# facebookresearch/generative-recommenders

Hardware: NVIDIA H100
Metric: user-seqs/sec HSTU-large L=8192 d=256 bf16 fwd+bwd (higher is better)
Workload: dtype bf16

## Files before the change

### generative_recommenders_b200/build.py

```python
import concurrent.futures
import importlib.util
import os
import shutil
import subprocess
import sys

HERE = os.path.dirname(os.path.abspath(__file__))
ROOT = os.path.dirname(HERE)
CSRC = os.path.join(HERE, "csrc")
OBJ = os.path.join(ROOT, "build", "hstu_b200")
LIB = os.path.join(HERE, "lib", "libhstu_b200.so")
SELFTEST_LIB = os.path.join(HERE, "lib", "libhstu_b200_selftest.so")
GEN = os.path.join(OBJ, "gen")
SELFTEST_SOURCES = ["wgmma_selftest.cu", "tmap.cu"]
SOURCES = ["api.cu", "attn_generic.cu", "attn_wgmma_fwd.cu", "attn_wgmma_bwd.cu", "attn_wgmma_fwd_e4m3.cu", "attn_wgmma_mixed_fwd.cu", "attn_wgmma_mixed_bwd.cu", "attn_fp16_operands.cu", "tmap.cu", "norm.cu", "norm_fast.cu", "jagged.cu", "position.cu", "sampled_softmax.cu", "jagged_bmm.cu"]
NVCC_FLAGS = [
    "-std=c++20", "-gencode", "arch=compute_90a,code=sm_90a", "-lineinfo", "-O3",
    "-Xcompiler", "-fPIC", "-Xcompiler", "-Wall", "-Xcudafe", "--diag_suppress=177",
]


def _nvcc() -> str:
    for cand in (os.environ.get("NVCC"), shutil.which("nvcc"), "/usr/local/cuda/bin/nvcc"):
        if cand and os.path.exists(cand):
            return cand
    raise RuntimeError("nvcc not found")


def _deps_mtime() -> float:
    paths = [os.path.join(CSRC, f) for f in os.listdir(CSRC)] + [os.path.join(ROOT, "include", "hstu_b200.h"), __file__,
# ... 64 lines not shown
```

### generative_recommenders_b200/csrc/attn_wgmma_bwd.cu

```cuda
#include "attn_wgmma_bwd.cuh"

namespace hstu {

template <int D, bool BF16>
__global__ void __launch_bounds__(kAttnThreads, 1) attn_bwd_wgmma_kernel(const __grid_constant__ BwdParams p) {
  bwd_key_tile<D, D, BF16, true>(p);
}

template <int D, bool BF16>
__global__ void __launch_bounds__(kAttnThreads, split_min_blocks(D)) attn_bwd_dkdv_wgmma_kernel(const __grid_constant__ BwdParams p) {
  bwd_key_tile<D, D, BF16, false>(p);
}

template <int D, bool BF16>
__global__ void __launch_bounds__(kAttnThreads, split_min_blocks(D)) attn_bwd_dq_wgmma_kernel(const __grid_constant__ BwdParams p) {
  bwd_dq_body<D, D, BF16>(p);
}

template <bool BF16>
__global__ void dq_convert_kernel(const float* __restrict__ acc, uint16_t* __restrict__ dq, long long rows, int heads, int D,
                                  long long row_stride, long long head_stride, float scale) {
  const long long nvec = rows * heads * (D / 8);
  for (long long idx = (long long)blockIdx.x * blockDim.x + threadIdx.x; idx < nvec; idx += (long long)gridDim.x * blockDim.x) {
    const int v = (int)(idx % (D / 8));
// ... 26 lines not shown
  hstu_attn_params q = p;
  if (q.out == nullptr) q.out = const_cast<void*>(q.q);
  q.o_row_stride = 8;
  q.o_head_stride = 8;
  return wgmma_bwd_supported(q);
}

static bool split_dq(const hstu_attn_params& p) {
  return p.dqk == 32 || p.dqk == 256 || p.dqk != p.dv || p.deterministic != 0;
}

static bool fp16_copies(const hstu_attn_params& p) { return p.dtype == HSTU_BF16 && p.dqk == 32 && p.dv == 32; }

size_t wgmma_workspace_bytes(const hstu_attn_params& p, bool bwd) {
  if (!bwd && p.delta_q_len > 0) return wgmma_delta_workspace_bytes(p);
  if (fp16_copies(p)) return fp16_operands_workspace_bytes(p, bwd);
  if (!bwd || split_dq(p)) return 0;
  return (size_t)p.total_rows * p.heads * p.dqk * sizeof(float);
}

template <int D, bool BF16, bool kSplit>
static int launch_bwd_wgmma(const hstu_attn_params& p, cudaStream_t st, const Fp16Operands* f16 = nullptr) {
  if constexpr (kSplit) {
    return launch_bwd_split<D, D, BF16>(p, st, attn_bwd_dkdv_wgmma_kernel<D, BF16>, attn_bwd_dq_wgmma_kernel<D, BF16>, f16);
  } else {
    using Cfg = BwdCfg<D, D, true>;
    const size_t need = wgmma_workspace_bytes(p, true);
    if (p.workspace == nullptr || p.workspace_bytes < need) {
      set_error("hstu_attn_bwd: workspace of %zu bytes required (got %zu)", need, p.workspace_bytes);
      return HSTU_ERR_WORKSPACE;
    }
    const BwdOperands o = bwd_operands(p, f16);
    BwdParams bp = bwd_params(p, f16);
    if (int e = make_tmap_rows_heads(&bp.tmQ, o.src[0], p.total_rows, p.heads, D, o.rs[0], o.hs[0], Cfg::BOX_COLS, Cfg::BQ)) return e;
    if (int e = make_tmap_rows_heads(&bp.tmK, o.src[1], p.total_rows, p.heads, D, o.rs[1], o.hs[1], Cfg::BOX_COLS, Cfg::BKV)) return e;
    if (int e = make_tmap_rows_heads(&bp.tmV, o.src[2], p.total_rows, p.heads, D, o.rs[2], o.hs[2], Cfg::BOX_COLS, Cfg::BKV)) return e;
    if (int e = make_tmap_rows_heads(&bp.tmDO, o.src[3], p.total_rows, p.heads, D, o.rs[3], o.hs[3], Cfg::BOX_COLS, Cfg::BQ)) return e;
    HSTU_CUDA_OK(cudaMemsetAsync(p.workspace, 0, need, st));
    auto kern = attn_bwd_wgmma_kernel<D, BF16>;
// ... 8 lines not shown
                                                         p.dq_row_stride, p.dq_head_stride, bp.dk_scale);
    HSTU_CUDA_OK(cudaGetLastError());
    return 0;
  }
}

int attn_wgmma_bwd(const hstu_attn_params& p, cudaStream_t st) {
  if (p.dqk != p.dv) return attn_wgmma_bwd_mixed(p, st);
  const bool bf = p.dtype == HSTU_BF16;
  const bool split = split_dq(p);
  switch (p.dqk) {
    case 32: {
      if (!bf) return launch_bwd_wgmma<32, false, true>(p, st);
      Fp16Operands f16;
      if (int e = fp16_operands_prepass(p, true, &f16, st)) return e;
      return launch_bwd_wgmma<32, false, true>(p, st, &f16);
    }
    case 64:
      if (split) return bf ? launch_bwd_wgmma<64, true, true>(p, st) : launch_bwd_wgmma<64, false, true>(p, st);
      return bf ? launch_bwd_wgmma<64, true, false>(p, st) : launch_bwd_wgmma<64, false, false>(p, st);
    case 128:
      if (split) return bf ? launch_bwd_wgmma<128, true, true>(p, st) : launch_bwd_wgmma<128, false, true>(p, st);
      return bf ? launch_bwd_wgmma<128, true, false>(p, st) : launch_bwd_wgmma<128, false, false>(p, st);
    case 256:
      return bf ? launch_bwd_wgmma<256, true, true>(p, st) : launch_bwd_wgmma<256, false, true>(p, st);
  }
  set_error("wgmma backward: unsupported head dim %d", p.dqk);
  return HSTU_ERR_UNSUPPORTED;
}

}
// ... 1 lines not shown
```

### generative_recommenders_b200/csrc/attn_wgmma_bwd.cuh

```cuda
#pragma once
#include <string.h>

#include <type_traits>

#include "attn_fp16_operands.cuh"
#include "attn_wgmma_qtile.cuh"
#include "common.cuh"
#include "internal.h"
#include "wgmma.cuh"

namespace hstu {
using namespace wg;

struct alignas(64) BwdParams {
  CUtensorMap tmQ, tmK, tmV, tmDO;
  SeqArgs seq;
  void* dk;
  void* dv;
  float* dq_acc;
  void* dq;
  long long dk_row_stride, dk_head_stride, dv_row_stride, dv_head_stride, dq_row_stride, dq_head_stride;
  float dv_scale;
  float dk_scale;
  const uint32_t* amax;
};

struct BwdScales {
  float c_s = 0.f, c_p = 1.f, c_d = 1.f;
  int e_dv = 0, e_dk = 0, e_dq = 0;
  __device__ __forceinline__ BwdScales(const BwdParams& p, int b, int h, int d) {
    c_s = p.seq.alpha_half;
    if (p.amax == nullptr) return;
    const OperandExps ex = operand_exps(p.amax + ((long long)b * p.seq.heads + h) * kAmaxSlots, 2.f * p.seq.alpha_half, d);
    c_s = ldexpf(p.seq.alpha_half, -(ex.q + ex.k));
    c_p = pow2f(ex.p);
    c_d = pow2f(ex.s - ex.v - ex.o);
    e_dv = -(ex.p + ex.o);
    e_dk = -(ex.s + ex.q);
    e_dq = -(ex.s + ex.k);
// ... 37 lines not shown
  uint64_t qd_full[4];
  uint32_t qd_free[4];
};

struct QTiles {
  int A, first, T;
  __device__ __forceinline__ int at(int i) const { return i < A ? i : first + (i - A); }
};

template <int DQK, int DV, bool BF16, bool FUSED_DQ>
__device__ __forceinline__ void bwd_key_tile(const BwdParams& p) {
  using Cfg = BwdCfg<DQK, DV, FUSED_DQ>;
  constexpr int SW = Cfg::SW, SWQ = Cfg::SWQ, SWV = Cfg::SWV, BQ = Cfg::BQ, NST = Cfg::STAGES;
  constexpr int NSL = Cfg::NSL, DNK = DQK / NSL, DNV = DV / NSL;
  static_assert(DNK % Cfg::BOX_COLS_Q == 0 && DNV % Cfg::BOX_COLS_V == 0, "a slice is whole boxes");
  const int b = blockIdx.z, h = blockIdx.y;
  const int n0 = (blockIdx.x / NSL) * Cfg::BKV;
  const int ck0 = (blockIdx.x % NSL) * DNK, cv0 = (blockIdx.x % NSL) * DNV;
  const long long row0 = load_index(p.seq.seq_offsets, p.seq.offsets_i64, b);
  int len = (int)(load_index(p.seq.seq_offsets, p.seq.offsets_i64, b + 1) - row0);
  if (len > p.seq.max_seq_len) {
    if (blockIdx.x == 0) {
      zero_rows(p.dk, 2, p.dk_row_stride, (long long)h * p.dk_head_stride, DQK, row0 + p.seq.max_seq_len, row0 + len);
      zero_rows(p.dv, 2, p.dv_row_stride, (long long)h * p.dv_head_stride, DV, row0 + p.seq.max_seq_len, row0 + len);
    }
    len = p.seq.max_seq_len;
  }
  if (n0 >= len) return;
  const int n_tgt = p.seq.num_targets ? (int)load_index(p.seq.num_targets, p.seq.targets_i64, b) : -1;
  const SeqMask msk = make_seq_mask(len, n_tgt, p.seq.win, p.seq.min_full, p.seq.ctx);
  const int nrows = min(Cfg::BKV, len - n0);
  QTiles qt;
  {
    int lo, hi, ctx_hi;
    q_range_for_kv_rows(msk, n0, n0 + nrows, &lo, &hi, &ctx_hi);
    qt.A = (ctx_hi + BQ - 1) / BQ;
    qt.first = max(lo / BQ, qt.A);
// ... 273 lines not shown
  static constexpr int STAGES = 3;
  static constexpr int OFF_Q = 0;
  static constexpr int OFF_DO = OFF_Q + Q_BYTES;
  static constexpr int OFF_K = OFF_DO + DO_BYTES;
  static constexpr int OFF_V = OFF_K + STAGES * K_BYTES;
  static constexpr int OFF_BAR = OFF_V + STAGES * V_BYTES;
  static constexpr int SMEM_BYTES = OFF_BAR + 256 + 1024;
  static_assert(SMEM_BYTES * split_min_blocks(DV) <= kSmemPerSm, "shared memory budget of split_min_blocks(dv) CTAs per SM");
};

template <int DQK, int DV, bool BF16>
__device__ __forceinline__ void bwd_dq_body(const BwdParams& p) {
  using Cfg = DqCfg<DQK, DV>;
  constexpr int SW = Cfg::SW, SWV = Cfg::SWV, BN = Cfg::BN, NST = Cfg::STAGES;
  constexpr bool kScaled = !BF16 && DQK == 32 && DV == 32;
  const int b = blockIdx.z, h = blockIdx.y;
  const int m0 = (int)(gridDim.x - 1 - blockIdx.x) * Cfg::BM;
  QTileSeq qs;
  if (!qtile_prologue<Cfg::BM, BN>(p.seq, b, h, m0, p.dq, p.dq_row_stride, p.dq_head_stride, DQK, &qs)) return;

  uint8_t* smem = dyn_smem_1k();
  KvRing<Cfg> ring{smem, &p.tmK, &p.tmV, h, qs.row0, qs.t0, qs.T};
  ring.init();
  const int tid = threadIdx.x, warp = tid >> 5, lane = tid & 31;
  if (tid == 0) {
    prefetch_tensormap(&p.tmQ);
    prefetch_tensormap(&p.tmK);
    prefetch_tensormap(&p.tmV);
    prefetch_tensormap(&p.tmDO);
    mbar_arrive_expect_tx(&ring.bars->q_full, Cfg::Q_BYTES + Cfg::DO_BYTES);
#pragma unroll
    for (int bx = 0; bx < imax(Cfg::NBOX, Cfg::NBOX_V); ++bx) {
      if (bx < Cfg::NBOX) tma_load_3d(smem + Cfg::OFF_Q + bx * Cfg::Q_BOX, &p.tmQ, &ring.bars->q_full, bx * Cfg::BOX_COLS, h, (int)(qs.row0 + m0));
      if (bx < Cfg::NBOX_V)
// ... 127 lines not shown
  bp.dq_acc = reinterpret_cast<float*>(p.workspace);
  bp.dq = p.dq;
  bp.dk_row_stride = p.dk_row_stride;
  bp.dk_head_stride = p.dk_head_stride;
  bp.dv_row_stride = p.dv_row_stride;
  bp.dv_head_stride = p.dv_head_stride;
  bp.dq_row_stride = p.dq_row_stride;
  bp.dq_head_stride = p.dq_head_stride;
  bp.dv_scale = 1.0f / (float)p.max_seq_len;
  bp.dk_scale = 0.5f * p.alpha / (float)p.max_seq_len;
  return bp;
}

template <int DQK, int DV, bool BF16>
int launch_bwd_split(const hstu_attn_params& p, cudaStream_t st, void (*kdkdv)(BwdParams), void (*kdq)(BwdParams),
                     const Fp16Operands* f16 = nullptr) {
  using Cfg = BwdCfg<DQK, DV, false>;
  const BwdOperands o = bwd_operands(p, f16);
  const int d[4] = {DQK, DQK, DV, DV};
  BwdParams bp = bwd_params(p, f16);
  if (int e = make_tmap_rows_heads(&bp.tmQ, o.src[0], p.total_rows, p.heads, d[0], o.rs[0], o.hs[0], Cfg::BOX_COLS_Q, Cfg::BQ)) return e;
  if (int e = make_tmap_rows_heads(&bp.tmK, o.src[1], p.total_rows, p.heads, d[1], o.rs[1], o.hs[1], Cfg::BOX_COLS, Cfg::BKV)) return e;
  if (int e = make_tmap_rows_heads(&bp.tmV, o.src[2], p.total_rows, p.heads, d[2], o.rs[2], o.hs[2], Cfg::BOX_COLS_V, Cfg::BKV)) return e;
  if (int e = make_tmap_rows_heads(&bp.tmDO, o.src[3], p.total_rows, p.heads, d[3], o.rs[3], o.hs[3], Cfg::BOX_COLS_V, Cfg::BQ)) return e;
  HSTU_CUDA_OK(cudaFuncSetAttribute(kdkdv, cudaFuncAttributeMaxDynamicSharedMemorySize, Cfg::SMEM_BYTES));
  const int key_ctas = (p.max_seq_len + Cfg::BKV - 1) / Cfg::BKV * Cfg::NSL;
  kdkdv<<<dim3(key_ctas, p.heads, p.batch), kAttnThreads, Cfg::SMEM_BYTES, st>>>(bp);
  HSTU_CUDA_OK(cudaGetLastError());
  using QC = DqCfg<DQK, DV>;
  if (int e = make_tmap_rows_heads(&bp.tmQ, o.src[0], p.total_rows, p.heads, d[0], o.rs[0], o.hs[0], QC::BOX_COLS, QC::BM)) return e;
  if (int e = make_tmap_rows_heads(&bp.tmK, o.src[1], p.total_rows, p.heads, d[1], o.rs[1], o.hs[1], QC::BOX_COLS, QC::BN)) return e;
  if (int e = make_tmap_rows_heads(&bp.tmV, o.src[2], p.total_rows, p.heads, d[2], o.rs[2], o.hs[2], QC::BOX_COLS_V, QC::BN)) return e;
  if (int e = make_tmap_rows_heads(&bp.tmDO, o.src[3], p.total_rows, p.heads, d[3], o.rs[3], o.hs[3], QC::BOX_COLS_V, QC::BM)) return e;
  HSTU_CUDA_OK(cudaFuncSetAttribute(kdq, cudaFuncAttributeMaxDynamicSharedMemorySize, QC::SMEM_BYTES));
  kdq<<<dim3((p.max_seq_len + QC::BM - 1) / QC::BM, p.heads, p.batch), kAttnThreads, QC::SMEM_BYTES, st>>>(bp);
  HSTU_CUDA_OK(cudaGetLastError());
  return 0;
}

}
```

### generative_recommenders_b200/csrc/attn_wgmma_fwd.cu

```cuda
#include "attn_wgmma_fwd.cuh"

namespace hstu {

template <int D, bool BF16>
__global__ void __launch_bounds__(kAttnThreads, kFwdMinBlocks<D>) attn_fwd_wgmma_kernel(const __grid_constant__ FwdParams p) {
  attn_fwd_wgmma_body<D, D, BF16, false>(p);
}
template <int D, bool BF16>
__global__ void __launch_bounds__(kAttnThreads, kFwdMinBlocks<D>) attn_fwd_delta_wgmma_kernel(const __grid_constant__ FwdParams p) {
  attn_fwd_wgmma_body<D, D, BF16, true>(p);
}

template <bool BF16>
__global__ void __launch_bounds__(256) delta_reduce_kernel(const float* __restrict__ part, void* out, long long rows, int heads, int d,
                                                            int chunks, long long o_row_stride, long long o_head_stride, float inv_n) {
  const long long plane = rows * heads * d, n4 = plane / 4;
  for (long long i = (long long)blockIdx.x * 256 + threadIdx.x; i < n4; i += (long long)gridDim.x * 256) {
    float4 a = reinterpret_cast<const float4*>(part)[i];
    for (int c = 1; c < chunks; ++c) {
      const float4 x = reinterpret_cast<const float4*>(part + c * plane)[i];
      a.x += x.x, a.y += x.y, a.z += x.z, a.w += x.w;
    }
    const long long e = i * 4, r = e / ((long long)heads * d), hc = e % ((long long)heads * d);
    const long long off = r * o_row_stride + (hc / d) * o_head_stride + hc % d;
// ... 43 lines not shown
    return false;
  return is_sm90();
}

int launch_delta_reduce(bool bf16, const float* part, void* out, long long rows, int heads, int d, int chunks,
                        long long o_row_stride, long long o_head_stride, float inv_n, cudaStream_t st) {
  const long long n4 = rows * heads * d / 4;
  const int blocks = (int)std::min<long long>((n4 + 255) / 256, kDeltaReduceBlocks);
  auto kern = bf16 ? delta_reduce_kernel<true> : delta_reduce_kernel<false>;
  kern<<<blocks, 256, 0, st>>>(part, out, rows, heads, d, chunks, o_row_stride, o_head_stride, inv_n);
  HSTU_CUDA_OK(cudaGetLastError());
  return 0;
}

template <int D, bool BF16, bool kDelta = false>
static int launch_fwd(const hstu_attn_params& p, cudaStream_t st, const Fp16Operands* f16 = nullptr) {
  auto kern = [] {
    if constexpr (kDelta) return attn_fwd_delta_wgmma_kernel<D, BF16>;
    else return attn_fwd_wgmma_kernel<D, BF16>;
  }();
  return launch_fwd_wgmma<D, D, BF16, kDelta>(p, st, kern, f16);
}

int attn_wgmma_fwd(const hstu_attn_params& p, cudaStream_t st) {
  if (p.dqk != p.dv) return attn_wgmma_fwd_mixed(p, st);
  const bool bf = p.dtype == HSTU_BF16;
  if (p.delta_q_len > 0) {
    switch (p.dqk) {
      case 32: return bf ? launch_fwd<32, true, true>(p, st) : launch_fwd<32, false, true>(p, st);
      case 64: return bf ? launch_fwd<64, true, true>(p, st) : launch_fwd<64, false, true>(p, st);
      case 128: return bf ? launch_fwd<128, true, true>(p, st) : launch_fwd<128, false, true>(p, st);
      case 256: return bf ? launch_fwd<256, true, true>(p, st) : launch_fwd<256, false, true>(p, st);
    }
  }
  switch (p.dqk) {
    case 32: {
      if (!bf) return launch_fwd<32, false>(p, st);
      Fp16Operands f16;
      if (int e = fp16_operands_prepass(p, false, &f16, st)) return e;
      return launch_fwd<32, false>(p, st, &f16);
    }
    case 64: return bf ? launch_fwd<64, true>(p, st) : launch_fwd<64, false>(p, st);
    case 128: return bf ? launch_fwd<128, true>(p, st) : launch_fwd<128, false>(p, st);
    case 256: return bf ? launch_fwd<256, true>(p, st) : launch_fwd<256, false>(p, st);
  }
  set_error("wgmma forward: unsupported head dim %d", p.dqk);
  return HSTU_ERR_UNSUPPORTED;
}

}
```

### generative_recommenders_b200/csrc/attn_wgmma_fwd.cuh

```cuda
#pragma once
#include <string.h>

#include <algorithm>
#include <type_traits>

#include "attn_fp16_operands.cuh"
#include "attn_wgmma_qtile.cuh"
#include "common.cuh"
#include "internal.h"
#include "wgmma.cuh"

namespace hstu {
using namespace wg;

struct alignas(64) FwdParams {
  CUtensorMap tmQ, tmK, tmV;
  SeqArgs seq;
  void* out;
  long long o_row_stride, o_head_stride;
  float inv_n;
  const uint32_t* amax;
  int delta;
  float* part;
};

template <int DQK, int DV = DQK>
struct FwdCfg {
  static constexpr int BM = 128;
  static constexpr int BN = 64;
  static constexpr int SW = swizzle_bytes(DQK), SWV = swizzle_bytes(DV);
  static constexpr int BOX_COLS = SW / 2;
  static constexpr int BOX_COLS_V = SWV / 2;
  static constexpr int Q_BOX = BM * SW;
  static constexpr int K_BOX = BN * SW;
  static constexpr int V_BOX = BN * SWV;
  static constexpr int Q_BYTES = BM * DQK * 2;
  static constexpr int K_BYTES = BN * DQK * 2;
  static constexpr int V_BYTES = BN * DV * 2;
// ... 14 lines not shown
  long long out_row, part_row;
  int rows;
};
template <int BM>
__device__ __forceinline__ DeltaRows delta_rows(const FwdParams& p) {
  const int m0 = (int)blockIdx.y * BM;
  const long long r = (long long)(blockIdx.x / p.seq.heads) * p.delta + m0;
  return {r, (long long)blockIdx.z * (gridDim.x / p.seq.heads) * p.delta + r, min(BM, p.delta - m0)};
}

template <int DQK, int DV, bool BF16, bool kDelta>
__device__ __forceinline__ void attn_fwd_wgmma_body(const FwdParams& p) {
  using Cfg = FwdCfg<DQK, DV>;
  constexpr int SW = Cfg::SW, SWV = Cfg::SWV, BN = Cfg::BN, NST = Cfg::STAGES;
  constexpr bool kMerge = DV <= 64;
  const int b = kDelta ? (int)blockIdx.x / p.seq.heads : (int)blockIdx.z, h = kDelta ? (int)blockIdx.x % p.seq.heads : (int)blockIdx.y;
  const int m0 = kDelta ? (int)blockIdx.y * Cfg::BM : (int)(gridDim.x - 1 - blockIdx.x) * Cfg::BM;
  QTileSeq qs;
  if constexpr (kDelta) {
    seq_rows(p.seq, b, &qs);
  } else if (!qtile_rows(p.seq, b, h, m0, p.out, p.o_row_stride, p.o_head_stride, DV, &qs)) {
    return;
  }
  const int p0 = kDelta ? qs.len - p.delta + m0 : m0;
  key_tiles<Cfg::BM, BN>(p.seq, b, p0, (kDelta ? p.delta : qs.len) - m0, &qs);
  if constexpr (kDelta) {
    const int per = (qs.T + (int)gridDim.z - 1) / (int)gridDim.z;
    qs.t0 += (int)blockIdx.z * per;
    qs.T = min(per, qs.T - (int)blockIdx.z * per);
    if (qs.T <= 0) {
      const DeltaRows dr = delta_rows<Cfg::BM>(p);
      for (int idx = threadIdx.x; idx < dr.rows * DV; idx += kAttnThreads) {
        if (gridDim.z > 1) p.part[((dr.part_row + idx / DV) * p.seq.heads + h) * DV + idx % DV] = 0.f;
        else reinterpret_cast<uint16_t*>(p.out)[(dr.out_row + idx / DV) * p.o_row_stride + (long long)h * p.o_head_stride + idx % DV] = 0;
      }
      return;
// ... 167 lines not shown
      for (int nb = 0; nb < DV / 8; ++nb) {
        float a = o[nb * 4 + hh * 2] * p.inv_n, c = o[nb * 4 + hh * 2 + 1] * p.inv_n;
        if (kScaled) a = scalbnf(a, e_out), c = scalbnf(c, e_out);
        *reinterpret_cast<uint32_t*>(orow + nb * 8 + 2 * t4) = out_bf16 ? pack_bf16x2(a, c) : pack_f16x2(a, c);
      }
    }
  }
}


int delta_chunks(const hstu_attn_params& p);
int launch_delta_reduce(bool bf16, const float* part, void* out, long long rows, int heads, int d, int chunks,
                        long long o_row_stride, long long o_head_stride, float inv_n, cudaStream_t st);

template <int DQK, int DV, bool BF16, bool kDelta>
int launch_fwd_wgmma(const hstu_attn_params& p, cudaStream_t st, void (*kern)(FwdParams), const Fp16Operands* f16 = nullptr) {
  using Cfg = FwdCfg<DQK, DV>;
  FwdParams fp;
  memset(&fp, 0, sizeof(fp));
  const int chunks = kDelta ? delta_chunks(p) : 1;
  if (chunks > 1) {
    const size_t need = wgmma_delta_workspace_bytes(p);
    if (p.workspace == nullptr || p.workspace_bytes < need) {
      set_error("hstu_attn_fwd: delta_q workspace of %zu bytes required (got %zu)", need, p.workspace_bytes);
      return HSTU_ERR_WORKSPACE;
    }
    fp.part = reinterpret_cast<float*>(p.workspace);
  }
  const long long q_rows = kDelta ? (long long)p.batch * p.delta_q_len : p.total_rows;
  if (f16) {
    const long long crs = (long long)p.heads * DQK, chs = DQK;
    if (int e = make_tmap_rows_heads(&fp.tmQ, f16->copy[0], p.total_rows, p.heads, DQK, crs, chs, Cfg::BOX_COLS, Cfg::BM)) return e;
    if (int e = make_tmap_rows_heads(&fp.tmK, f16->copy[1], p.total_rows, p.heads, DQK, crs, chs, Cfg::BOX_COLS, Cfg::BN)) return e;
    if (int e = make_tmap_rows_heads(&fp.tmV, f16->copy[2], p.total_rows, p.heads, DV, crs, chs, Cfg::BOX_COLS_V, Cfg::BN)) return e;
    fp.amax = f16->amax;
  } else {
    if (int e = make_tmap_rows_heads(&fp.tmQ, p.q, q_rows, p.heads, DQK, p.q_row_stride, p.q_head_stride, Cfg::BOX_COLS, Cfg::BM)) return e;
    if (int e = make_tmap_rows_heads(&fp.tmK, p.k, p.total_rows, p.heads, DQK, p.k_row_stride, p.k_head_stride, Cfg::BOX_COLS, Cfg::BN)) return e;
    if (int e = make_tmap_rows_heads(&fp.tmV, p.v, p.total_rows, p.heads, DV, p.v_row_stride, p.v_head_stride, Cfg::BOX_COLS_V, Cfg::BN)) return e;
  }
  fp.seq = seq_args(p);
  fp.out = p.out;
  fp.o_row_stride = p.o_row_stride;
  fp.o_head_stride = p.o_head_stride;
  fp.inv_n = 1.0f / (float)p.max_seq_len;
  fp.delta = p.delta_q_len;
  HSTU_CUDA_OK(cudaFuncSetAttribute(kern, cudaFuncAttributeMaxDynamicSharedMemorySize, Cfg::SMEM_BYTES));
  const dim3 grid = kDelta ? dim3(p.batch * p.heads, (p.delta_q_len + Cfg::BM - 1) / Cfg::BM, chunks)
                           : dim3((p.max_seq_len + Cfg::BM - 1) / Cfg::BM, p.heads, p.batch);
  kern<<<grid, kAttnThreads, Cfg::SMEM_BYTES, st>>>(fp);
  HSTU_CUDA_OK(cudaGetLastError());
  if (chunks > 1) return launch_delta_reduce(BF16, fp.part, p.out, q_rows, p.heads, DV, chunks, p.o_row_stride, p.o_head_stride, fp.inv_n, st);
  return 0;
}

}
```

### generative_recommenders_b200/csrc/attn_wgmma_qtile.cuh

```cuda
#pragma once
#include <type_traits>

#include "common.cuh"
#include "internal.h"
#include "wgmma.cuh"

namespace hstu {
using namespace wg;

constexpr int kAttnThreads = 256;

struct SeqArgs {
  const void* seq_offsets;
  const void* num_targets;
  int offsets_i64, targets_i64;
  int max_seq_len, heads;
  int win, min_full, ctx;
  float alpha_half;
};
inline SeqArgs seq_args(const hstu_attn_params& p) {
  return {p.seq_offsets,  p.num_targets,           p.offsets_are_i64,    p.num_targets_are_i64, p.max_seq_len, p.heads,
          p.max_attn_len, p.min_full_attn_seq_len, p.contextual_seq_len, 0.5f * p.alpha};
}

struct QTileSeq {
  long long row0;
  int len, mrows, t0, T;
  SeqMask msk;
};
__device__ __forceinline__ void seq_rows(const SeqArgs& a, int b, QTileSeq* q) {
  const long long row0 = load_index(a.seq_offsets, a.offsets_i64, b);
  q->len = (int)(load_index(a.seq_offsets, a.offsets_i64, b + 1) - row0);
  q->row0 = row0;
}
__device__ __forceinline__ bool qtile_rows(const SeqArgs& a, int b, int h, int m0, void* out, long long row_stride,
                                           long long head_stride, int d, QTileSeq* q) {
  seq_rows(a, b, q);
  if (q->len > a.max_seq_len) {
    if (blockIdx.x == 0) zero_rows(out, 2, row_stride, (long long)h * head_stride, d, q->row0 + a.max_seq_len, q->row0 + q->len);
    q->len = a.max_seq_len;
  }
  return m0 < q->len;
}

template <int BM, int BN>
__device__ __forceinline__ void key_tiles(const SeqArgs& a, int b, int p0, int rows, QTileSeq* q) {
  const int n_tgt = a.num_targets ? (int)load_index(a.num_targets, a.targets_i64, b) : -1;
  q->msk = make_seq_mask(q->len, n_tgt, a.win, a.min_full, a.ctx);
  q->mrows = min(BM, rows);
  int lo, hi;
  kv_range_for_q_rows(q->msk, p0, p0 + q->mrows, &lo, &hi);
  q->t0 = lo / BN;
  q->T = (hi + BN - 1) / BN - q->t0;
}
template <int BM, int BN>
__device__ __forceinline__ bool qtile_prologue(const SeqArgs& a, int b, int h, int m0, void* out, long long row_stride,
                                               long long head_stride, int d, QTileSeq* q) {
  if (!qtile_rows(a, b, h, m0, out, row_stride, head_stride, d, q)) return false;
  key_tiles<BM, BN>(a, b, m0, q->len - m0, q);
  return true;
}

struct QTileBars {
  uint64_t q_full;
  uint64_t k_full[3], v_full[3];
  uint32_t k_free[3], v_free[3];
};
constexpr std::false_type kKey{};
constexpr std::true_type kVal{};

template <class Cfg>
struct KvRing {
  static_assert(Cfg::STAGES <= 3, "QTileBars holds three stages");
// ... 83 lines not shown
```

### generative_recommenders_b200/csrc/common.cuh

```cuda
#pragma once
#include <cuda_bf16.h>
#include <cuda_fp16.h>
#include <cuda_runtime.h>
#include <stdint.h>
#include <stdio.h>

#include "../../include/hstu_b200.h"

namespace hstu {

void set_error(const char* fmt, ...);

#define HSTU_CHECK_ARG(cond, ...)            \
  do {                                       \
    if (!(cond)) {                           \
      ::hstu::set_error(__VA_ARGS__);        \
      return HSTU_ERR_INVALID_ARGUMENT;      \
    }                                        \
  } while (0)

#define HSTU_CUDA_OK(expr)                                                              \
  do {                                                                                  \
    cudaError_t _e = (expr);                                                            \
    if (_e != cudaSuccess) {                                                            \
// ... 106 lines not shown
      long long last = (long long)idl + m.win + (m.ctx > 0 ? m.ctx - 1 : 0) + 1;
      if (last < h) h = (int)last;
    }
    if (h < n1) h = n1 < m.len ? n1 : m.len;
  }
  int c = 0;
  if (m.ctx > 0) {
    c = m.ctx < l ? m.ctx : l;
    if (c > m.len) c = m.len;
  }
  *lo = l;
  *hi = h;
  *ctx_hi = c;
}

__device__ __forceinline__ long long load_index(const void* p, int is_i64, int idx) {
  return is_i64 ? (long long)reinterpret_cast<const long long*>(p)[idx] : (long long)reinterpret_cast<const int*>(p)[idx];
}

__device__ __forceinline__ void zero_rows(void* base, int elem_bytes, long long row_stride, long long head_off, int d,
                                          long long r0, long long r1) {
  const long long n = (r1 - r0) * d;
  for (long long idx = threadIdx.x; idx < n; idx += blockDim.x) {
    const long long r = r0 + idx / d, c = idx % d;
    const long long off = r * row_stride + head_off + c;
    if (elem_bytes == 2) reinterpret_cast<uint16_t*>(base)[off] = 0;
    else reinterpret_cast<uint32_t*>(base)[off] = 0u;
  }
}

// ... 13 lines not shown
```

### generative_recommenders_b200/csrc/internal.h

```cpp
#pragma once
#include <cuda_runtime.h>
#include <stddef.h>

#include "../../include/hstu_b200.h"

namespace hstu {
void set_error(const char* fmt, ...);

int attn_generic_fwd(const hstu_attn_params& p, cudaStream_t st);
int attn_generic_bwd(const hstu_attn_params& p, cudaStream_t st);

bool wgmma_supported(const hstu_attn_params& p, bool bwd);
size_t wgmma_workspace_bytes(const hstu_attn_params& p, bool bwd);
int attn_wgmma_fwd(const hstu_attn_params& p, cudaStream_t st);
int attn_wgmma_bwd(const hstu_attn_params& p, cudaStream_t st);
int attn_wgmma_fwd_mixed(const hstu_attn_params& p, cudaStream_t st);
int attn_wgmma_bwd_mixed(const hstu_attn_params& p, cudaStream_t st);
bool aligned_view(const void* ptr, long long row_stride, long long head_stride);
bool wgmma_fwd_supported(const hstu_attn_params& p);
size_t wgmma_delta_workspace_bytes(const hstu_attn_params& p);

struct Fp16Operands {
  const unsigned int* amax;
  const void* copy[4];
};
size_t fp16_operands_workspace_bytes(const hstu_attn_params& p, bool bwd);
int fp16_operands_prepass(const hstu_attn_params& p, bool bwd, Fp16Operands* out, cudaStream_t st);
size_t e4m3_v_copy_bytes(const hstu_attn_params& p);
int e4m3_v_prepass(const hstu_attn_params& p, const void** v16, cudaStream_t st);

int e4m3_fwd_check(const hstu_attn_params& p);
int attn_wgmma_fwd_e4m3(const hstu_attn_params& p, const hstu_attn_descales& ds, cudaStream_t st);
bool is_sm90();

int layer_norm_fwd(const void* x, const void* w, const void* b, void* y, float* mean, float* rstd, long long n, int D,
                   long long xs, long long ys, float eps, int dtype, int swish, bool rms, cudaStream_t st);
int layer_norm_bwd(const void* dy, const void* x, const void* w, const void* b, const float* mean, const float* rstd,
                   void* dx, float* dw, float* db, float* partial, long long n, int D, long long xs, long long dys,
                   long long dxs, int dtype, int swish, bool rms, cudaStream_t st);
int norm_mul_dropout_fwd(const void* attn, const void* u, const void* w, const void* b, void* out, float* mean,
                         float* rstd, long long n, int H, int dv, long long as, long long us, float eps, float p,
                         unsigned long long seed, int dtype, int silu_u, int concat, int gn, cudaStream_t st);
// ... 45 lines not shown
```

### generative_recommenders_b200/ops/hstu_attention.py

```python
import ctypes as C
from typing import Optional, Tuple

import torch

from .. import _lib
from ..common import HammerKernel, require_cuda_kernel, switch_to_contiguous_if_needed


def _fill_common(p, max_seq_len, alpha, q, k, v, seq_offsets, num_targets, max_attn_len, contextual_seq_len,
                 min_full_attn_seq_len, impl, delta_q_len=0):
    if seq_offsets.dtype not in (torch.int32, torch.int64):
        raise RuntimeError("seq_offsets must be int32 or int64")
    if num_targets is not None and num_targets.dtype not in (torch.int32, torch.int64):
        raise RuntimeError("num_targets must be int32 or int64")
    p.abi_version = _lib.ABI_VERSION
    p.dtype = _lib.dtype_code(q)
    p.impl = impl
    p.batch = seq_offsets.numel() - 1
    p.heads = q.shape[1]
    p.dqk = q.shape[2]
    p.dv = v.shape[2]
    p.max_seq_len = int(max_seq_len)
    p.total_rows = k.shape[0]
    p.alpha = float(alpha)
# ... 45 lines not shown
        num_targets = num_targets.contiguous()
    if out is None:
        out = torch.empty((q.shape[0], q.shape[1], v.shape[2]), dtype=v.dtype, device=dev)
    p = _lib.AttnParams()
    _fill_common(p, max_seq_len, alpha, q, k, v, seq_offsets, num_targets, max_attn_len, contextual_seq_len,
                 min_full_attn_seq_len, impl, delta_q_len)
    p.out = out.data_ptr()
    p.o_row_stride, p.o_head_stride = out.stride(0), out.stride(1)
    keep = _fill_bias(p, bias, None)
    ws = _workspace(p, False, dev)
    with torch.cuda.device(dev), _lib.timed("attn_fwd", dev):
        _lib.check(_lib.lib().hstu_attn_fwd(C.byref(p), _lib.stream_ptr(dev)), "hstu_attn_fwd")
    if delta_q_len:
        _lib.note_launch(2 if ws is not None else 1)
    else:
        _lib.note_launch(3 if ws is not None else 1)
    del ws, keep
    return out


_FP8 = torch.float8_e4m3fn


def cuda_hstu_attention_fwd_fp8(
    max_seq_len: int, alpha: float, q: torch.Tensor, k: torch.Tensor, v: torch.Tensor, seq_offsets: torch.Tensor,
    descales: Optional[Tuple[Optional[torch.Tensor], Optional[torch.Tensor], Optional[torch.Tensor]]] = None,
    num_targets: Optional[torch.Tensor] = None, max_attn_len: int = 0, contextual_seq_len: int = 0,
    min_full_attn_seq_len: int = 0, impl: int = _lib.IMPL_AUTO, out: Optional[torch.Tensor] = None,
) -> torch.Tensor:
    if not all(t.dtype == _FP8 for t in (q, k, v)):
        raise RuntimeError(f"fp8 attention: q, k and v must all be torch.float8_e4m3fn (got {q.dtype}, {k.dtype}, {v.dtype}); "
# ... 53 lines not shown
    if num_targets is not None:
        num_targets = num_targets.contiguous()
    p = _lib.AttnParams()
    _fill_common(p, max_seq_len, alpha, q, k, v, seq_offsets, num_targets, max_attn_len, contextual_seq_len,
                 min_full_attn_seq_len, impl)
    p.dout, p.dq, p.dk, p.dv_out = dout.data_ptr(), dq.data_ptr(), dk.data_ptr(), dv.data_ptr()
    p.do_row_stride, p.do_head_stride = dout.stride(0), dout.stride(1)
    p.dq_row_stride, p.dq_head_stride = dq.stride(0), dq.stride(1)
    p.dk_row_stride, p.dk_head_stride = dk.stride(0), dk.stride(1)
    p.dv_row_stride, p.dv_head_stride = dv.stride(0), dv.stride(1)
    p.deterministic = int(bool(deterministic))
    keep = _fill_bias(p, bias, dbias)
    ws = _workspace(p, True, dev)
    with torch.cuda.device(dev), _lib.timed("attn_bwd", dev):
        _lib.check(_lib.lib().hstu_attn_bwd(C.byref(p), _lib.stream_ptr(dev)), "hstu_attn_bwd")
    _lib.note_launch(4 if ws is not None and p.dtype == _lib.BF16 and p.dqk == 32 else 2)
    del ws, keep


def _fill_bias(p, bias, dbias):
    if bias is None:
        return None
    pos_w, ts_w, timestamps = bias
    keep = []
    n, B = int(p.max_seq_len), int(p.batch)
    if pos_w is not None and pos_w.numel() != 2 * n - 1:
        raise RuntimeError(f"relative position bias: pos_w must have 2 * max_seq_len - 1 = {2 * n - 1} entries, got {pos_w.numel()}")
    if (ts_w is None) != (timestamps is None):
        raise RuntimeError("relative time bias: ts_w and timestamps must be given together")
    if ts_w is not None:
        if tuple(timestamps.shape) != (B, n):
# ... 127 lines not shown
```

Measured before the change: 103.0.

## Schedule head-dim-32 query tiles longest-first via a device-side cost sort

Adds a small single-CTA kernel that estimates each query tile's key-tile count from the sequence mask, bucket-sorts tiles per batch by descending cost, and writes an order list. The forward and dQ kernels then launch a flat grid and read (batch, head, tile) from that list, so the heaviest tiles are scheduled first for better tail balance on jagged, masked sequences. The dK/dV kernel grid is also reordered so heads vary fastest for a key tile. The cost is one extra launch per fwd and bwd plus extra workspace, and the path only applies to the bf16 head-dim-32 fp16-copy route.

```diff
diff --git a/generative_recommenders_b200/build.py b/generative_recommenders_b200/build.py
--- a/generative_recommenders_b200/build.py
+++ b/generative_recommenders_b200/build.py
@@ -13,7 +13,7 @@
 SELFTEST_LIB = os.path.join(HERE, "lib", "libhstu_b200_selftest.so")
 GEN = os.path.join(OBJ, "gen")
 SELFTEST_SOURCES = ["wgmma_selftest.cu", "tmap.cu"]
-SOURCES = ["api.cu", "attn_generic.cu", "attn_wgmma_fwd.cu", "attn_wgmma_bwd.cu", "attn_wgmma_fwd_e4m3.cu", "attn_wgmma_mixed_fwd.cu", "attn_wgmma_mixed_bwd.cu", "attn_fp16_operands.cu", "tmap.cu", "norm.cu", "norm_fast.cu", "jagged.cu", "position.cu", "sampled_softmax.cu", "jagged_bmm.cu"]
+SOURCES = ["api.cu", "attn_generic.cu", "attn_wgmma_fwd.cu", "attn_wgmma_bwd.cu", "attn_wgmma_fwd_e4m3.cu", "attn_wgmma_mixed_fwd.cu", "attn_wgmma_mixed_bwd.cu", "attn_fp16_operands.cu", "attn_order.cu", "tmap.cu", "norm.cu", "norm_fast.cu", "jagged.cu", "position.cu", "sampled_softmax.cu", "jagged_bmm.cu"]
 NVCC_FLAGS = [
     "-std=c++20", "-gencode", "arch=compute_90a,code=sm_90a", "-lineinfo", "-O3",
     "-Xcompiler", "-fPIC", "-Xcompiler", "-Wall", "-Xcudafe", "--diag_suppress=177",
diff --git a/generative_recommenders_b200/csrc/attn_order.cu b/generative_recommenders_b200/csrc/attn_order.cu
--- /dev/null
+++ b/generative_recommenders_b200/csrc/attn_order.cu
@@ -0,0 +1,99 @@
+#include "attn_wgmma_bwd.cuh"
+#include "attn_wgmma_fwd.cuh"
+
+namespace hstu {
+
+namespace {
+
+constexpr int kOrderThreads = 1024, kOrderWarps = kOrderThreads / 32;
+constexpr int kOrderBuckets = 512;
+constexpr int kTileRows = 128, kKeyRows = 64;
+static_assert(FwdCfg<32>::BM == kTileRows && FwdCfg<32>::BN == kKeyRows, "forward tiles");
+static_assert(DqCfg<32, 32>::BM == kTileRows && DqCfg<32, 32>::BN == kKeyRows, "dQ tiles (one list with the forward)");
+
+struct OrderParams {
+  SeqArgs seq;
+  int batch, tiles;
+  int nb;
+  int2* items;
+};
+
+__global__ void __launch_bounds__(kOrderThreads) attn_order_kernel(const __grid_constant__ OrderParams p) {
+  extern __shared__ int cnt[];
+  const int warp = threadIdx.x >> 5, lane = threadIdx.x & 31;
+  const unsigned lt = (1u << lane) - 1u;
+  int* own = cnt + warp * p.nb;
+  for (int b = warp; b < p.batch; b += kOrderWarps) {
+    const long long row0 = load_index(p.seq.seq_offsets, p.seq.offsets_i64, b);
+    const int len = (int)min(load_index(p.seq.seq_offsets, p.seq.offsets_i64, b + 1) - row0, (long long)p.seq.max_seq_len);
+    const int n_tgt = p.seq.num_targets ? (int)load_index(p.seq.num_targets, p.seq.targets_i64, b) : -1;
+    const SeqMask msk = make_seq_mask(len, n_tgt, p.seq.win, p.seq.min_full, p.seq.ctx);
+    const int ne = len > 0 ? (len + kTileRows - 1) / kTileRows : 0;
+    auto cost = [&](int t) {
+      const int r0 = t * kTileRows;
+      return min(key_tiles_of_q_rows<kKeyRows>(msk, r0, min(kTileRows, len - r0)).T, p.nb - 1);
+    };
+    for (int c = lane; c < p.nb; c += 32) own[c] = 0;
+    __syncwarp();
+    for (int t = lane; t < ne; t += 32) atomicAdd(&own[cost(t)], 1);
+    __syncwarp();
+    int run = 0;
+    for (int top = p.nb - 1; top >= 0; top -= 32) {
+      const int c = top - lane;
+      const int v = c >= 0 ? own[c] : 0;
+      int incl = v;
+#pragma unroll
+      for (int o = 1; o < 32; o <<= 1) {
+        const int y = __shfl_up_sync(0xffffffffu, incl, o);
+        if (lane >= o) incl += y;
+      }
+      if (c >= 0) own[c] = run + incl - v;
+      run += __shfl_sync(0xffffffffu, incl, 31);
+    }
+    __syncwarp();
+    for (int t0 = 0; t0 < ne; t0 += 32) {
+      const int t = t0 + lane;
+      const int c = t < ne ? cost(t) : -1;
+      const unsigned peers = __match_any_sync(0xffffffffu, c);
+      const int pos = c >= 0 ? own[c] + __popc(peers & lt) : 0;
+      __syncwarp();
+      if (c >= 0 && (peers & lt) == 0u) own[c] += __popc(peers);
+      __syncwarp();
+      if (c >= 0) p.items[b * p.tiles + pos] = make_int2(t, b);
+    }
+    for (int t = ne + lane; t < p.tiles; t += 32) p.items[b * p.tiles + t] = make_int2(-1, -1);
+    __syncwarp();
+  }
+}
+
+}
+
+static size_t align256(size_t n) { return (n + 255) / 256 * 256; }
+
+static int order_items(const hstu_attn_params& p) { return p.batch * ((p.max_seq_len + kTileRows - 1) / kTileRows); }
+
+size_t attn_order_bytes(const hstu_attn_params& p) { return align256((size_t)order_items(p) * sizeof(int2)); }
+
+int attn_order(const hstu_attn_params& p, size_t offset, const int2** items, cudaStream_t st) {
+  const size_t need = offset + attn_order_bytes(p);
+  if (p.workspace == nullptr || p.workspace_bytes < need) {
+    set_error("hstu_attn: workspace of %zu bytes required (got %zu)", need, p.workspace_bytes);
+    return HSTU_ERR_WORKSPACE;
+  }
+  OrderParams op;
+  op.seq = seq_args(p);
+  op.batch = p.batch;
+  op.tiles = (p.max_seq_len + kTileRows - 1) / kTileRows;
+  const char* unsorted = getenv("HSTU_ATTN_UNSORTED");
+  op.nb = unsorted != nullptr && unsorted[0] == '1' ? 1 : std::min((p.max_seq_len + kKeyRows - 1) / kKeyRows + 1, kOrderBuckets);
+  op.items = reinterpret_cast<int2*>(static_cast<uint8_t*>(p.workspace) + offset);
+  *items = op.items;
+  if (order_items(p) == 0) return 0;
+  const int smem = kOrderWarps * op.nb * (int)sizeof(int);
+  HSTU_CUDA_OK(cudaFuncSetAttribute(attn_order_kernel, cudaFuncAttributeMaxDynamicSharedMemorySize, smem));
+  attn_order_kernel<<<1, kOrderThreads, smem, st>>>(op);
+  HSTU_CUDA_OK(cudaGetLastError());
+  return 0;
+}
+
+}
diff --git a/generative_recommenders_b200/csrc/attn_wgmma_bwd.cu b/generative_recommenders_b200/csrc/attn_wgmma_bwd.cu
--- a/generative_recommenders_b200/csrc/attn_wgmma_bwd.cu
+++ b/generative_recommenders_b200/csrc/attn_wgmma_bwd.cu
@@ -64,15 +64,16 @@
 
 size_t wgmma_workspace_bytes(const hstu_attn_params& p, bool bwd) {
   if (!bwd && p.delta_q_len > 0) return wgmma_delta_workspace_bytes(p);
-  if (fp16_copies(p)) return fp16_operands_workspace_bytes(p, bwd);
+  if (fp16_copies(p)) return fp16_operands_workspace_bytes(p, bwd) + attn_order_bytes(p);
   if (!bwd || split_dq(p)) return 0;
   return (size_t)p.total_rows * p.heads * p.dqk * sizeof(float);
 }
 
 template <int D, bool BF16, bool kSplit>
-static int launch_bwd_wgmma(const hstu_attn_params& p, cudaStream_t st, const Fp16Operands* f16 = nullptr) {
+static int launch_bwd_wgmma(const hstu_attn_params& p, cudaStream_t st, const Fp16Operands* f16 = nullptr,
+                            const int2* order = nullptr) {
   if constexpr (kSplit) {
-    return launch_bwd_split<D, D, BF16>(p, st, attn_bwd_dkdv_wgmma_kernel<D, BF16>, attn_bwd_dq_wgmma_kernel<D, BF16>, f16);
+    return launch_bwd_split<D, D, BF16>(p, st, attn_bwd_dkdv_wgmma_kernel<D, BF16>, attn_bwd_dq_wgmma_kernel<D, BF16>, f16, order);
   } else {
     using Cfg = BwdCfg<D, D, true>;
     const size_t need = wgmma_workspace_bytes(p, true);
@@ -111,7 +112,9 @@
       if (!bf) return launch_bwd_wgmma<32, false, true>(p, st);
       Fp16Operands f16;
       if (int e = fp16_operands_prepass(p, true, &f16, st)) return e;
-      return launch_bwd_wgmma<32, false, true>(p, st, &f16);
+      const int2* order;
+      if (int e = attn_order(p, fp16_operands_workspace_bytes(p, true), &order, st)) return e;
+      return launch_bwd_wgmma<32, false, true>(p, st, &f16, order);
     }
     case 64:
       if (split) return bf ? launch_bwd_wgmma<64, true, true>(p, st) : launch_bwd_wgmma<64, false, true>(p, st);
diff --git a/generative_recommenders_b200/csrc/attn_wgmma_bwd.cuh b/generative_recommenders_b200/csrc/attn_wgmma_bwd.cuh
--- a/generative_recommenders_b200/csrc/attn_wgmma_bwd.cuh
+++ b/generative_recommenders_b200/csrc/attn_wgmma_bwd.cuh
@@ -23,6 +23,7 @@
   float dv_scale;
   float dk_scale;
   const uint32_t* amax;
+  const int2* order;
 };
 
 struct BwdScales {
@@ -90,13 +91,15 @@
   constexpr int SW = Cfg::SW, SWQ = Cfg::SWQ, SWV = Cfg::SWV, BQ = Cfg::BQ, NST = Cfg::STAGES;
   constexpr int NSL = Cfg::NSL, DNK = DQK / NSL, DNV = DV / NSL;
   static_assert(DNK % Cfg::BOX_COLS_Q == 0 && DNV % Cfg::BOX_COLS_V == 0, "a slice is whole boxes");
-  const int b = blockIdx.z, h = blockIdx.y;
-  const int n0 = (blockIdx.x / NSL) * Cfg::BKV;
+  constexpr bool kHeadsInner = !FUSED_DQ && DQK == 32 && DV == 32;
+  static_assert(!kHeadsInner || NSL == 1, "one CTA per key tile");
+  const int b = blockIdx.z, h = kHeadsInner ? blockIdx.x : blockIdx.y;
+  const int n0 = ((kHeadsInner ? blockIdx.y : blockIdx.x) / NSL) * Cfg::BKV;
   const int ck0 = (blockIdx.x % NSL) * DNK, cv0 = (blockIdx.x % NSL) * DNV;
   const long long row0 = load_index(p.seq.seq_offsets, p.seq.offsets_i64, b);
   int len = (int)(load_index(p.seq.seq_offsets, p.seq.offsets_i64, b + 1) - row0);
   if (len > p.seq.max_seq_len) {
-    if (blockIdx.x == 0) {
+    if ((kHeadsInner ? blockIdx.y : blockIdx.x) == 0) {
       zero_rows(p.dk, 2, p.dk_row_stride, (long long)h * p.dk_head_stride, DQK, row0 + p.seq.max_seq_len, row0 + len);
       zero_rows(p.dv, 2, p.dv_row_stride, (long long)h * p.dv_head_stride, DV, row0 + p.seq.max_seq_len, row0 + len);
     }
@@ -400,10 +403,19 @@
   using Cfg = DqCfg<DQK, DV>;
   constexpr int SW = Cfg::SW, SWV = Cfg::SWV, BN = Cfg::BN, NST = Cfg::STAGES;
   constexpr bool kScaled = !BF16 && DQK == 32 && DV == 32;
-  const int b = blockIdx.z, h = blockIdx.y;
-  const int m0 = (int)(gridDim.x - 1 - blockIdx.x) * Cfg::BM;
+  constexpr bool kOrder = DQK == 32 && DV == 32;
+  int b, h, m0;
+  if constexpr (kOrder) {
+    int tile;
+    if (!cta_work(p.order, p.seq.heads, (int)(gridDim.x - 1 - blockIdx.x), &b, &h, &tile)) return;
+    m0 = tile * Cfg::BM;
+  } else {
+    b = blockIdx.z, h = blockIdx.y;
+    m0 = (int)(gridDim.x - 1 - blockIdx.x) * Cfg::BM;
+  }
   QTileSeq qs;
-  if (!qtile_prologue<Cfg::BM, BN>(p.seq, b, h, m0, p.dq, p.dq_row_stride, p.dq_head_stride, DQK, &qs)) return;
+  if (!qtile_prologue<Cfg::BM, BN>(p.seq, b, h, m0, kOrder ? m0 == 0 : blockIdx.x == 0, p.dq, p.dq_row_stride, p.dq_head_stride, DQK, &qs))
+    return;
 
   uint8_t* smem = dyn_smem_1k();
   KvRing<Cfg> ring{smem, &p.tmK, &p.tmV, h, qs.row0, qs.t0, qs.T};
@@ -561,7 +573,7 @@
 
 template <int DQK, int DV, bool BF16>
 int launch_bwd_split(const hstu_attn_params& p, cudaStream_t st, void (*kdkdv)(BwdParams), void (*kdq)(BwdParams),
-                     const Fp16Operands* f16 = nullptr) {
+                     const Fp16Operands* f16 = nullptr, const int2* order = nullptr) {
   using Cfg = BwdCfg<DQK, DV, false>;
   const BwdOperands o = bwd_operands(p, f16);
   const int d[4] = {DQK, DQK, DV, DV};
@@ -572,7 +584,8 @@
   if (int e = make_tmap_rows_heads(&bp.tmDO, o.src[3], p.total_rows, p.heads, d[3], o.rs[3], o.hs[3], Cfg::BOX_COLS_V, Cfg::BQ)) return e;
   HSTU_CUDA_OK(cudaFuncSetAttribute(kdkdv, cudaFuncAttributeMaxDynamicSharedMemorySize, Cfg::SMEM_BYTES));
   const int key_ctas = (p.max_seq_len + Cfg::BKV - 1) / Cfg::BKV * Cfg::NSL;
-  kdkdv<<<dim3(key_ctas, p.heads, p.batch), kAttnThreads, Cfg::SMEM_BYTES, st>>>(bp);
+  const dim3 key_grid = DQK == 32 && DV == 32 ? dim3(p.heads, key_ctas, p.batch) : dim3(key_ctas, p.heads, p.batch);
+  kdkdv<<<key_grid, kAttnThreads, Cfg::SMEM_BYTES, st>>>(bp);
   HSTU_CUDA_OK(cudaGetLastError());
   using QC = DqCfg<DQK, DV>;
   if (int e = make_tmap_rows_heads(&bp.tmQ, o.src[0], p.total_rows, p.heads, d[0], o.rs[0], o.hs[0], QC::BOX_COLS, QC::BM)) return e;
@@ -580,7 +593,9 @@
   if (int e = make_tmap_rows_heads(&bp.tmV, o.src[2], p.total_rows, p.heads, d[2], o.rs[2], o.hs[2], QC::BOX_COLS_V, QC::BN)) return e;
   if (int e = make_tmap_rows_heads(&bp.tmDO, o.src[3], p.total_rows, p.heads, d[3], o.rs[3], o.hs[3], QC::BOX_COLS_V, QC::BM)) return e;
   HSTU_CUDA_OK(cudaFuncSetAttribute(kdq, cudaFuncAttributeMaxDynamicSharedMemorySize, QC::SMEM_BYTES));
-  kdq<<<dim3((p.max_seq_len + QC::BM - 1) / QC::BM, p.heads, p.batch), kAttnThreads, QC::SMEM_BYTES, st>>>(bp);
+  const int q_ctas = (p.max_seq_len + QC::BM - 1) / QC::BM;
+  bp.order = order;
+  kdq<<<order ? dim3(q_ctas * p.heads * p.batch) : dim3(q_ctas, p.heads, p.batch), kAttnThreads, QC::SMEM_BYTES, st>>>(bp);
   HSTU_CUDA_OK(cudaGetLastError());
   return 0;
 }
diff --git a/generative_recommenders_b200/csrc/attn_wgmma_fwd.cu b/generative_recommenders_b200/csrc/attn_wgmma_fwd.cu
--- a/generative_recommenders_b200/csrc/attn_wgmma_fwd.cu
+++ b/generative_recommenders_b200/csrc/attn_wgmma_fwd.cu
@@ -81,12 +81,12 @@
 }
 
 template <int D, bool BF16, bool kDelta = false>
-static int launch_fwd(const hstu_attn_params& p, cudaStream_t st, const Fp16Operands* f16 = nullptr) {
+static int launch_fwd(const hstu_attn_params& p, cudaStream_t st, const Fp16Operands* f16 = nullptr, const int2* order = nullptr) {
   auto kern = [] {
     if constexpr (kDelta) return attn_fwd_delta_wgmma_kernel<D, BF16>;
     else return attn_fwd_wgmma_kernel<D, BF16>;
   }();
-  return launch_fwd_wgmma<D, D, BF16, kDelta>(p, st, kern, f16);
+  return launch_fwd_wgmma<D, D, BF16, kDelta>(p, st, kern, f16, order);
 }
 
 int attn_wgmma_fwd(const hstu_attn_params& p, cudaStream_t st) {
@@ -105,7 +105,9 @@
       if (!bf) return launch_fwd<32, false>(p, st);
       Fp16Operands f16;
       if (int e = fp16_operands_prepass(p, false, &f16, st)) return e;
-      return launch_fwd<32, false>(p, st, &f16);
+      const int2* order;
+      if (int e = attn_order(p, fp16_operands_workspace_bytes(p, false), &order, st)) return e;
+      return launch_fwd<32, false>(p, st, &f16, order);
     }
     case 64: return bf ? launch_fwd<64, true>(p, st) : launch_fwd<64, false>(p, st);
     case 128: return bf ? launch_fwd<128, true>(p, st) : launch_fwd<128, false>(p, st);
diff --git a/generative_recommenders_b200/csrc/attn_wgmma_fwd.cuh b/generative_recommenders_b200/csrc/attn_wgmma_fwd.cuh
--- a/generative_recommenders_b200/csrc/attn_wgmma_fwd.cuh
+++ b/generative_recommenders_b200/csrc/attn_wgmma_fwd.cuh
@@ -22,6 +22,7 @@
   const uint32_t* amax;
   int delta;
   float* part;
+  const int2* order;
 };
 
 template <int DQK, int DV = DQK>
@@ -66,12 +67,21 @@
   using Cfg = FwdCfg<DQK, DV>;
   constexpr int SW = Cfg::SW, SWV = Cfg::SWV, BN = Cfg::BN, NST = Cfg::STAGES;
   constexpr bool kMerge = DV <= 64;
-  const int b = kDelta ? (int)blockIdx.x / p.seq.heads : (int)blockIdx.z, h = kDelta ? (int)blockIdx.x % p.seq.heads : (int)blockIdx.y;
-  const int m0 = kDelta ? (int)blockIdx.y * Cfg::BM : (int)(gridDim.x - 1 - blockIdx.x) * Cfg::BM;
+  constexpr bool kOrder = !kDelta && DQK == 32 && DV == 32;
+  int b, h, m0;
+  if constexpr (kOrder) {
+    int tile;
+    if (!cta_work(p.order, p.seq.heads, (int)(gridDim.x - 1 - blockIdx.x), &b, &h, &tile)) return;
+    m0 = tile * Cfg::BM;
+  } else {
+    b = kDelta ? (int)blockIdx.x / p.seq.heads : (int)blockIdx.z;
+    h = kDelta ? (int)blockIdx.x % p.seq.heads : (int)blockIdx.y;
+    m0 = kDelta ? (int)blockIdx.y * Cfg::BM : (int)(gridDim.x - 1 - blockIdx.x) * Cfg::BM;
+  }
   QTileSeq qs;
   if constexpr (kDelta) {
     seq_rows(p.seq, b, &qs);
-  } else if (!qtile_rows(p.seq, b, h, m0, p.out, p.o_row_stride, p.o_head_stride, DV, &qs)) {
+  } else if (!qtile_rows(p.seq, b, h, m0, kOrder ? m0 == 0 : blockIdx.x == 0, p.out, p.o_row_stride, p.o_head_stride, DV, &qs)) {
     return;
   }
   const int p0 = kDelta ? qs.len - p.delta + m0 : m0;
@@ -269,7 +279,8 @@
                         long long o_row_stride, long long o_head_stride, float inv_n, cudaStream_t st);
 
 template <int DQK, int DV, bool BF16, bool kDelta>
-int launch_fwd_wgmma(const hstu_attn_params& p, cudaStream_t st, void (*kern)(FwdParams), const Fp16Operands* f16 = nullptr) {
+int launch_fwd_wgmma(const hstu_attn_params& p, cudaStream_t st, void (*kern)(FwdParams), const Fp16Operands* f16 = nullptr,
+                     const int2* order = nullptr) {
   using Cfg = FwdCfg<DQK, DV>;
   FwdParams fp;
   memset(&fp, 0, sizeof(fp));
@@ -300,9 +311,12 @@
   fp.o_head_stride = p.o_head_stride;
   fp.inv_n = 1.0f / (float)p.max_seq_len;
   fp.delta = p.delta_q_len;
+  fp.order = order;
   HSTU_CUDA_OK(cudaFuncSetAttribute(kern, cudaFuncAttributeMaxDynamicSharedMemorySize, Cfg::SMEM_BYTES));
+  const int tiles = (p.max_seq_len + Cfg::BM - 1) / Cfg::BM;
   const dim3 grid = kDelta ? dim3(p.batch * p.heads, (p.delta_q_len + Cfg::BM - 1) / Cfg::BM, chunks)
-                           : dim3((p.max_seq_len + Cfg::BM - 1) / Cfg::BM, p.heads, p.batch);
+                    : order ? dim3(tiles * p.heads * p.batch)
+                            : dim3(tiles, p.heads, p.batch);
   kern<<<grid, kAttnThreads, Cfg::SMEM_BYTES, st>>>(fp);
   HSTU_CUDA_OK(cudaGetLastError());
   if (chunks > 1) return launch_delta_reduce(BF16, fp.part, p.out, q_rows, p.heads, DV, chunks, p.o_row_stride, p.o_head_stride, fp.inv_n, st);
diff --git a/generative_recommenders_b200/csrc/attn_wgmma_qtile.cuh b/generative_recommenders_b200/csrc/attn_wgmma_qtile.cuh
--- a/generative_recommenders_b200/csrc/attn_wgmma_qtile.cuh
+++ b/generative_recommenders_b200/csrc/attn_wgmma_qtile.cuh
@@ -33,11 +33,26 @@
   q->len = (int)(load_index(a.seq_offsets, a.offsets_i64, b + 1) - row0);
   q->row0 = row0;
 }
-__device__ __forceinline__ bool qtile_rows(const SeqArgs& a, int b, int h, int m0, void* out, long long row_stride,
+__device__ __forceinline__ bool cta_work(const int2* order, int heads, int grid_tile, int* b, int* h, int* tile) {
+  if (order != nullptr) {
+    const int i = (int)blockIdx.x / heads;
+    const int2 it = order[i];
+    *b = it.y;
+    *h = (int)blockIdx.x - i * heads;
+    *tile = it.x;
+    return it.x >= 0;
+  }
+  *b = (int)blockIdx.z;
+  *h = (int)blockIdx.y;
+  *tile = grid_tile;
+  return true;
+}
+
+__device__ __forceinline__ bool qtile_rows(const SeqArgs& a, int b, int h, int m0, bool zero_owner, void* out, long long row_stride,
                                            long long head_stride, int d, QTileSeq* q) {
   seq_rows(a, b, q);
   if (q->len > a.max_seq_len) {
-    if (blockIdx.x == 0) zero_rows(out, 2, row_stride, (long long)h * head_stride, d, q->row0 + a.max_seq_len, q->row0 + q->len);
+    if (zero_owner) zero_rows(out, 2, row_stride, (long long)h * head_stride, d, q->row0 + a.max_seq_len, q->row0 + q->len);
     q->len = a.max_seq_len;
   }
   return m0 < q->len;
@@ -48,15 +63,14 @@
   const int n_tgt = a.num_targets ? (int)load_index(a.num_targets, a.targets_i64, b) : -1;
   q->msk = make_seq_mask(q->len, n_tgt, a.win, a.min_full, a.ctx);
   q->mrows = min(BM, rows);
-  int lo, hi;
-  kv_range_for_q_rows(q->msk, p0, p0 + q->mrows, &lo, &hi);
-  q->t0 = lo / BN;
-  q->T = (hi + BN - 1) / BN - q->t0;
+  const KeyTiles kt = key_tiles_of_q_rows<BN>(q->msk, p0, q->mrows);
+  q->t0 = kt.t0;
+  q->T = kt.T;
 }
 template <int BM, int BN>
-__device__ __forceinline__ bool qtile_prologue(const SeqArgs& a, int b, int h, int m0, void* out, long long row_stride,
+__device__ __forceinline__ bool qtile_prologue(const SeqArgs& a, int b, int h, int m0, bool zero_owner, void* out, long long row_stride,
                                                long long head_stride, int d, QTileSeq* q) {
-  if (!qtile_rows(a, b, h, m0, out, row_stride, head_stride, d, q)) return false;
+  if (!qtile_rows(a, b, h, m0, zero_owner, out, row_stride, head_stride, d, q)) return false;
   key_tiles<BM, BN>(a, b, m0, q->len - m0, q);
   return true;
 }
diff --git a/generative_recommenders_b200/csrc/common.cuh b/generative_recommenders_b200/csrc/common.cuh
--- a/generative_recommenders_b200/csrc/common.cuh
+++ b/generative_recommenders_b200/csrc/common.cuh
@@ -144,6 +144,16 @@
   *ctx_hi = c;
 }
 
+struct KeyTiles {
+  int t0, T;
+};
+template <int BN>
+__host__ __device__ inline KeyTiles key_tiles_of_q_rows(const SeqMask& m, int p0, int rows) {
+  int lo, hi;
+  kv_range_for_q_rows(m, p0, p0 + rows, &lo, &hi);
+  return {lo / BN, (hi + BN - 1) / BN - lo / BN};
+}
+
 __device__ __forceinline__ long long load_index(const void* p, int is_i64, int idx) {
   return is_i64 ? (long long)reinterpret_cast<const long long*>(p)[idx] : (long long)reinterpret_cast<const int*>(p)[idx];
 }
diff --git a/generative_recommenders_b200/csrc/internal.h b/generative_recommenders_b200/csrc/internal.h
--- a/generative_recommenders_b200/csrc/internal.h
+++ b/generative_recommenders_b200/csrc/internal.h
@@ -26,6 +26,8 @@
 };
 size_t fp16_operands_workspace_bytes(const hstu_attn_params& p, bool bwd);
 int fp16_operands_prepass(const hstu_attn_params& p, bool bwd, Fp16Operands* out, cudaStream_t st);
+size_t attn_order_bytes(const hstu_attn_params& p);
+int attn_order(const hstu_attn_params& p, size_t offset, const int2** items, cudaStream_t st);
 size_t e4m3_v_copy_bytes(const hstu_attn_params& p);
 int e4m3_v_prepass(const hstu_attn_params& p, const void** v16, cudaStream_t st);
 
diff --git a/generative_recommenders_b200/ops/hstu_attention.py b/generative_recommenders_b200/ops/hstu_attention.py
--- a/generative_recommenders_b200/ops/hstu_attention.py
+++ b/generative_recommenders_b200/ops/hstu_attention.py
@@ -83,7 +83,7 @@
     if delta_q_len:
         _lib.note_launch(2 if ws is not None else 1)
     else:
-        _lib.note_launch(3 if ws is not None else 1)
+        _lib.note_launch(4 if ws is not None else 1)
     del ws, keep
     return out
 
@@ -167,7 +167,7 @@
     ws = _workspace(p, True, dev)
     with torch.cuda.device(dev), _lib.timed("attn_bwd", dev):
         _lib.check(_lib.lib().hstu_attn_bwd(C.byref(p), _lib.stream_ptr(dev)), "hstu_attn_bwd")
-    _lib.note_launch(4 if ws is not None and p.dtype == _lib.BF16 and p.dqk == 32 else 2)
+    _lib.note_launch(5 if ws is not None and p.dtype == _lib.BF16 and p.dqk == 32 else 2)
     del ws, keep
 
 
```

After: 104.2, median of 6. 1.01x the previous value.
